# HKUST-Aerial-Robotics/ESVO

Measured on AMD Instinct MI355X. Metric: mapped events/sec (stereo TS raster + block matching + LM depth refinement + fusion), events resident in HBM before the timed region; exactly K ticks between two synchronisations, i.e. including the fill and the drain of the two-deep tick pipeline (`sustained`: the same workload over 1600 ticks), higher is better.
Workload: dtype f64

## Files before the change

### esvo_amd/csrc/api_core.hip

```cpp
#include "context.hpp"

namespace esvo_host {
thread_local std::string g_create_error;
}

namespace {

void invert3x3(const double* P, double* Kinv, double* Kinv_t) {
  const double a = P[0], b = P[1], cc = P[2], d = P[4], e = P[5], f = P[6], g = P[8], hh = P[9], i = P[10];
  const double det = a * (e * i - f * hh) - b * (d * i - f * g) + cc * (d * hh - e * g);
  const double id = 1.0 / det;
  Kinv[0] = (e * i - f * hh) * id; Kinv[1] = (cc * hh - b * i) * id; Kinv[2] = (b * f - cc * e) * id;
  Kinv[3] = (f * g - d * i) * id;  Kinv[4] = (a * i - cc * g) * id;  Kinv[5] = (cc * d - a * f) * id;
  Kinv[6] = (d * hh - e * g) * id; Kinv[7] = (b * g - a * hh) * id;  Kinv[8] = (a * e - b * d) * id;
  for (int r = 0; r < 3; ++r) Kinv_t[r] = (Kinv[r * 3 + 0] * P[3] + Kinv[r * 3 + 1] * P[7]) + Kinv[r * 3 + 2] * P[11];
}

int validate_params(const esvo_params_t* p, std::string& why) {
  if (p->ls_norm != ESVO_LSNORM_TDIST && p->ls_norm != ESVO_LSNORM_L2) { why = "LSnorm must be Tdist or l2 (DepthProblemSolver.cpp:121-131 exits on anything else)"; return ESVO_ERR_UNSUPPORTED; }
  if (p->bm_step < 1) { why = "BM_step must be >= 1"; return ESVO_ERR_INVALID_ARG; }
  if (p->patch_size_x < 1 || p->patch_size_x > 64 || p->patch_size_y < 1 || p->patch_size_y > 40) { why = "patch size must be within 1..64 x 1..40"; return ESVO_ERR_UNSUPPORTED; }
  if (p->median_blur_kernel_size < 0 || p->median_blur_kernel_size > 3) { why = "median_blur_kernel_size must be 0..3 (kernel 2k + 1)"; return ESVO_ERR_UNSUPPORTED; }
  if (p->max_event_queue_len < 0 || p->max_event_queue_len > TSQ_LMAX) { why = "max_event_queue_len must be 0 (one stamp per pixel) or 1..32"; return ESVO_ERR_UNSUPPORTED; }
  if (p->bm_max_disparity < p->bm_min_disparity || p->bm_min_disparity < 0) { why = "bad disparity range"; return ESVO_ERR_INVALID_ARG; }
// ... 20 lines not shown
  const double td_stdvar = std::sqrt(p.td_nu / (p.td_nu - 2) * (p.td_scale * p.td_scale));
  d.td_stdvar2 = td_stdvar * td_stdvar;
  d.lm_max_iter = p.lm_max_iteration; d.lm_maxfev = p.lm_max_iteration * 3;
  d.invdepth_min = p.invdepth_min; d.invdepth_max = p.invdepth_max;
  d.var_thr = p.stdvar_vis_threshold * p.stdvar_vis_threshold;
  d.cost_thr = (p.residual_vis_threshold * p.residual_vis_threshold) * (double)(p.patch_size_x * p.patch_size_y);
  d.age_thr = p.age_vis_threshold;
  d.fusion_radius = p.fusion_radius;
  d.reg_radius = p.reg_radius; d.reg_min_nb = p.reg_min_neighbours; d.reg_min_close = p.reg_min_close_neighbours;
  d.num_threads = p.num_threads;
  d.ls_norm = p.ls_norm;
}

template <typename T>
hipError_t dalloc(T** p, size_t n) { return hipMalloc(reinterpret_cast<void**>(p), (n ? n : 1) * sizeof(T)); }

void set_compute_band(esvo_context* h) {
  const int halo = 2 + (h->prm.regularization ? h->prm.reg_radius : 0);
  h->dp.cband_y0 = std::max(0, h->dp.band_y0 - halo);
  h->dp.cband_y1 = std::min(h->H, h->dp.band_y1 + halo);
}

void release_routing(esvo_context* h) {
  for (int cam = 0; cam < 2; ++cam) {
    if (h->h_route_ev[cam]) hipHostFree(h->h_route_ev[cam]);
    h->h_route_ev[cam] = nullptr;
    h->route_cap[cam] = 0;
  }
  if (h->h_route_gidx) hipHostFree(h->h_route_gidx);
  h->h_route_gidx = nullptr;
// ... 224 lines not shown
  CK(hipMalloc(reinterpret_cast<void**>(&h->d_map), map_buffer_bytes(npx)));
  CK(hipMalloc(reinterpret_cast<void**>(&h->d_map2), map_buffer_bytes(npx)));
  CK(hipMemset(h->d_map, 0, map_buffer_bytes(npx)));
  CK(hipMemset(h->d_map2, 0, map_buffer_bytes(npx)));
  h->d_map_cur = h->d_map;
  CK(dalloc(&h->d_owner_max, npx));
  CK(dalloc(&h->d_owner_min, npx));
  CK(dalloc(&h->d_own_w, E));
  CK(dalloc(&h->d_lkeep, E));
  h->codes_bytes = (E + 7) / 8 * 8;
  CK(dalloc(&h->d_codes, h->codes_bytes));
  CK(dalloc(&h->d_sel, E));
  CK(dalloc(&h->d_evmap, npx + 64));
  CK(dalloc(&h->d_reg_ab, npx));
  CK(dalloc(&h->d_reg_cd, npx));
  CK(dalloc(&h->d_exp_flags, npx));
  CK(dalloc(&h->d_exp_prefix, npx));
  CK(dalloc(&h->d_export, npx));
  CK(dalloc(&h->d_export_cell, npx));
  for (int i = 0; i < EV_N; ++i) CK(hipEventCreate(&h->evt[i]));
  if (h->tl_on) { CK(hipEventCreate(&h->tl_ref)); CK(hipEventRecord(h->tl_ref, h->stream)); CK(hipEventSynchronize(h->tl_ref)); }
  h->evt_ok = true;
  CK(hipEventCreateWithFlags(&h->evt_trk_read, hipEventDisableTiming));
  for (int cam = 0; cam < 2; ++cam) CK(hipEventCreateWithFlags(&h->evt_ingest[cam], hipEventDisableTiming));
  CK(hipHostMalloc(reinterpret_cast<void**>(&h->h_pose_pool), sizeof(double) * 16 * (size_t)h->max_poses * esvo_context::POSE_POOL));
  for (int i = 0; i < esvo_context::POSE_POOL; ++i) CK(hipEventCreate(&h->pool_evt[i]));
  h->pool_ok = true;
  for (int i = 0; i < 16; ++i) h->T_world_obs[i] = h->T_world_frame[i] = (i % 5 == 0) ? 1.0 : 0.0;
#undef CK
  *out = h;
// ... 4 lines not shown
  if (!h) return ESVO_OK;
  hipSetDevice(h->device);
  if (h->stream) hipStreamSynchronize(h->stream);
  if (h->stream_l) hipStreamSynchronize(h->stream_l);
  if (h->stream_l1) hipStreamSynchronize(h->stream_l1);
  if (h->stream_b) hipStreamSynchronize(h->stream_b);
  comm_release(h);
  em_release(h);
  void* ptrs[] = {h->d_lut, h->d_mask, h->d_fixmap[0], h->d_fixmap[1], h->d_sae[0], h->d_sae[1], h->d_raw, h->d_raw1, h->d_fwd_lut[0], h->d_fwd_lut[1], h->d_fwd_off[0], h->d_fwd_off[1],
                  h->d_fwd_src[0], h->d_fwd_src[1], h->d_fwd_val, h->d_ts[0],
                  h->d_ts[1], h->d_ring[0], h->d_ring[1], h->d_obs2[0][0], h->d_obs2[0][1], h->d_obs2[1][0], h->d_obs2[1][1], h->d_obs_tmp,
                  h->d_pose_T2[0], h->d_pose_T2[1], h->d_scan_tmp_b, h->d_cnt_b, h->d_tick_ev, h->d_match_slots, h->d_match_flags, h->d_match_prefix,
                  h->d_matches2[0], h->d_matches2[1], h->d_scan_tmp_l2[0], h->d_scan_tmp_l2[1], h->d_pt_slots2[0], h->d_pt_slots2[1], h->d_pt_flags2[0], h->d_pt_flags2[1], h->d_pt_prefix2[0], h->d_pt_prefix2[1], h->d_pts_tmp, h->d_stage[0], h->d_stage[1], h->d_counters2[0], h->d_counters2[1], h->d_scan_tmp,
                  h->d_win, h->d_frame_pose_T, h->d_fr_table, h->d_prop, h->d_tile_pts, h->d_tile_count, h->d_over_pts,
                  h->d_cell_count, h->d_cell_offset, h->d_cell_list, h->d_fuse_ctr, h->d_rec_ids, h->d_map, h->d_map2, h->d_owner_max, h->d_owner_min, h->d_exp_flags,
                  h->d_exp_prefix, h->d_export, h->d_export_cell, h->d_reg_ab, h->d_reg_cd, h->d_tsq[0], h->d_tsq[1], h->d_tsq_tcount, h->d_tsq_tlist, h->d_tsq_over, h->d_tsq_over_count, h->d_own_w, h->d_lkeep, h->d_codes, h->d_codes_send, h->d_codes_all, h->d_pts_send, h->d_pts_all, h->d_rank_kept,
                  h->d_sel, h->d_evmap, h->d_lm_fvec0, h->d_lm_fnorm0, h->d_lm_meta, h->d_lm_order, h->d_lm_hist, h->d_clk, h->d_ring_gidx, h->d_halo_viol, h->d_dn_flags, h->d_merge_a, h->d_merge_b, h->d_merge_plan, h->d_tsq_dup};
  for (void* p : ptrs) if (p) hipFree(p);
  if (h->h_counters) hipHostFree(h->h_counters);
  if (h->h_cnt_b) hipHostFree(h->h_cnt_b);
  if (h->h_pin) hipHostFree(h->h_pin);
  if (h->h_fr_table) hipHostFree(h->h_fr_table);
  if (h->evt_ok) for (int i = 0; i < EV_N; ++i) hipEventDestroy(h->evt[i]);
  if (h->pool_ok) for (int i = 0; i < esvo_context::POSE_POOL; ++i) hipEventDestroy(h->pool_evt[i]);
  if (h->h_pose_pool) hipHostFree(h->h_pose_pool);
  if (h->h_trk_ne) hipHostFree(h->h_trk_ne);
  if (h->h_trk_xyz) hipHostFree(h->h_trk_xyz);
  release_routing(h);
  for (int cam = 0; cam < 2; ++cam) if (h->d_wire[cam]) hipFree(h->d_wire[cam]);
  if (h->evt_trk_read) hipEventDestroy(h->evt_trk_read);
  if (h->tl_ref) hipEventDestroy(h->tl_ref);
// ... 101 lines not shown
    const u32 need = params->fusion_strategy == ESVO_FUSION_CONST_POINTS ? (u32)(1.5 * params->max_fusion_points) + 4u
                                                                         : (u32)params->max_fusion_frames + 2u;
    if (need > h->max_frames) FAIL(ESVO_ERR_CAPACITY, "fusion window (frames) exceeds the capacity fixed at esvo_create");
  }
  if (h->routed && (params->smooth_time_surface != h->prm.smooth_time_surface || params->median_blur_kernel_size != h->prm.median_blur_kernel_size ||
                    params->patch_size_y != h->prm.patch_size_y || params->denoising != h->prm.denoising || params->bm_updown))
    FAIL(ESVO_ERR_STATE, "the handle routes events by row (esvo_shard_set_routing): SmoothTimeSurface, median_blur_kernel_size, patch_size_Y and Denoising "
                         "fix the rows it renders and the events it keeps; esvo_reset + esvo_shard_set_routing to change them");
  esvo_params_t np = *params;
  np.max_events_per_tick = h->prm.max_events_per_tick;
  np.max_window_points = h->prm.max_window_points;
  np.max_poses_per_tick = h->prm.max_poses_per_tick;
  np.event_ring_capacity = h->prm.event_ring_capacity;
  if (np.max_event_queue_len != h->prm.max_event_queue_len) FAIL(ESVO_ERR_CAPACITY, "max_event_queue_len is fixed at esvo_create (the per-pixel queues are allocated there)");
  h->prm = np;
  fill_dev_params(h);
  set_compute_band(h);
  return ESVO_OK;
}

int esvo_set_stream(esvo_handle h, void* hip_stream) {
  if (!h) return ESVO_ERR_INVALID_ARG;
  API_LOCK(h);
  std::lock_guard<std::mutex> lp0(h->mu_push[0]), lp1(h->mu_push[1]);
  { int rcp = flush_pending_tick(h); if (rcp) return rcp; }
  HIPCHK(hipStreamSynchronize(h->stream));
  HIPCHK(hipStreamSynchronize(h->stream_l)); HIPCHK(hipStreamSynchronize(h->stream_l1));
  HIPCHK(hipStreamSynchronize(h->stream_b));
  if (h->own_stream && h->stream) hipStreamDestroy(h->stream);
  h->stream = reinterpret_cast<hipStream_t>(hip_stream);
// ... 107 lines not shown
```

### esvo_amd/csrc/api_map.hip

```cpp
#include <chrono>

#include "context.hpp"

namespace esvo_host {

u64 lower_bound_sec(const esvo_context* h, int cam, double t) {
  const auto& v = h->ts_host[cam];
  size_t lo = 0, hi = v.size();
  while (lo < hi) {
    size_t mid = (lo + hi) / 2;
    if (ns_to_sec(v[mid]) < t) lo = mid + 1; else hi = mid;
  }
  return h->ring_base[cam] + lo;
}
u64 ros_time_from_sec(double t) {
  long long sec64 = (long long)std::floor(t);
  u32 sec = (u32)sec64;
  u32 nsec = (u32)std::round((t - sec) * 1e9);
  sec += (nsec / 1000000000ul);
  nsec %= 1000000000ul;
  return (u64)sec * 1000000000ull + nsec;
}

int upload_poses(esvo_context* h, const uint64_t* pose_t_ns, const double* pose_T, size_t m, u32* d_zero_row = nullptr) {
// ... 347 lines not shown
  if (total > h->win_cap) {
    for (int e : tail_ev) if (e >= 0) hipEventRecord(h->evt[e], sb);
    FAIL(ESVO_ERR_CAPACITY, "window points exceed capacity");
  }
  const int o = par * EV_BACK_STRIDE;
  const bool timed = h->stage_events_on;
  h->back_timed[par] = timed;
  if (timed) hipEventRecord(h->evt[EV_FU0 + o], sb);
  launch_fuse(a, h->dp, sb);
  if (timed) hipEventRecord(h->evt[EV_FU1 + o], sb);
  h->d_map_cur = h->d_map;
  const bool do_clean = naive ? false : (h->prm.clean_requires_full_window ? (h->n_window_frames >= (size_t)h->prm.max_fusion_frames) : true);
  if (do_clean) launch_clean(h->d_map, h->dp, sb);
  if (timed) hipEventRecord(h->evt[EV_CL1 + o], sb);
  if (h->prm.regularization && !naive) {
    launch_reg_view(h->d_map, h->d_map2, h->d_owner_max, h->d_owner_min, h->d_reg_ab, h->d_reg_cd, h->d_cnt_b + 7, h->dp, sb);
    const u64 band_cells = (u64)std::max(h->dp.band_y1 - h->dp.band_y0, 1) * (u64)h->W;
    const bool sparse = h->reg_sparse_forced >= 0 ? h->reg_sparse_forced == 1 : (u64)h->stats.last_map_size * 10u < band_cells;
    launch_reg_apply(h->d_map, h->d_map2, h->d_owner_max, h->d_owner_min, h->d_reg_ab, h->d_reg_cd, h->d_cnt_b + 7, h->dp, sb, sparse);
    h->d_map_cur = h->d_map2;
  }
  HIPCHK(hipMemcpyAsync(h->h_cnt_b + 8 * par, h->d_cnt_b, sizeof(u32) * 8, hipMemcpyDeviceToHost, sb));
  if (h->routed) HIPCHK(hipMemcpyAsync(h->h_cnt_b + 8 * 3 + par, h->d_halo_viol, sizeof(u32), hipMemcpyDeviceToHost, sb));
  hipEventRecord(h->evt[EV_RG1 + o], sb);
  for (int e : tail_ev) if (e >= 0) hipEventRecord(h->evt[e], sb);
  HIPCHK(hipGetLastError());
  h->back_pending[par] = true;
  return ESVO_OK;
}

int export_map(esvo_context* h, std::vector<esvo_depth_point_t>& out, std::vector<u32>* cells) {
  launch_map_compact(h->d_map_cur, h->d_exp_flags, h->d_exp_prefix, h->d_cnt_b + 5, h->d_scan_tmp_b, h->d_export,
                     h->d_export_cell, h->dp, h->stream_b);
  int rc = read_counters_b(h, 2, true);
// ... 1394 lines not shown
```

### esvo_amd/csrc/common.hpp

```cpp
#pragma once

#include <hip/hip_runtime.h>
#include <stdint.h>

#include "../../include/esvo_hip.h"

#define ESVO_WAVE 64

#include <cstdlib>
#include <cstring>
inline const char* esvo_dev_switch(const char* name) {
  const char* on = std::getenv("ESVO_DEV_SWITCHES");
  return (on && std::strcmp(on, "1") == 0) ? std::getenv(name) : nullptr;
}

namespace esvo {

typedef unsigned long long u64;
typedef unsigned int u32;

struct CamConst {
  double P[12];
  double Kinv[9];
  double Kinv_t[3];
// ... 284 lines not shown
  u32* class_count;
  u32* class_total;
  u32 lds_cap;
  u32 pmax_plus1;
  u32* d_total;
  MapCell* map;
  u32* d_num_fusion;
  u32* n_touched;
  int naive;
  u32* owner_max;
  u32* owner_min;
  u32* n_reg_elems;
};
void launch_fuse(const FuseArgs& a, const DevParams& p, hipStream_t s);
void launch_clean(MapCell* map, const DevParams& p, hipStream_t s);
void launch_reg_view(const MapCell* map_in, MapCell* map_out, u32* owner_max, u32* owner_min, double2* ab, double2* cd,
                     u32* n_elems, const DevParams& p, hipStream_t s);
void launch_reg_apply(const MapCell* map_in, MapCell* map_out, const u32* owner_max, const u32* owner_min, const double2* ab,
                      const double2* cd, u32* n_elems, const DevParams& p, hipStream_t s, bool sparse = false);
struct SgmScratch {
  uint8_t *sobL, *rawL, *sobR, *rawR;
  int16_t* vol[6];
  int16_t *d1, *d1b;
  u32* d2key;
};
void launch_sgbm(const uint8_t* left, const uint8_t* right, const SgmScratch& s, int16_t* disp, int W, int H, hipStream_t st);
void launch_sgm_points(const esvo_event_t* ring, u64 first, u64 cap, u32 n, const float2* lut, const int16_t* disp, DevPoint* slots,
                       u32* flags, const DevParams& p, hipStream_t st);
void launch_sgm_naive(const DevPoint* pts, u32 n, const double* d_T_frame_obs, u32* owner, u32* pair_flags, u32* pair_rank, u32* d_total,
                      u32* scan_tmp, MapCell* map, const DevParams& p, hipStream_t st);
void launch_debug_image(const MapCell* map, u32* owner, uint8_t* bgr, const uint8_t* jet, int type, double max_range,
                        double min_range, double thr1, double thr2, const DevParams& p, hipStream_t s);
void launch_map_compact(const MapCell* map, u32* flags, u32* prefix, u32* d_total, u32* scan_tmp,
                        esvo_depth_point_t* out, u32* out_cell, const DevParams& p, hipStream_t s);
// ... 3 lines not shown
```

### esvo_amd/csrc/context.hpp

```cpp
#pragma once
#include <algorithm>
#include <array>
#include <atomic>
#include <chrono>
#include <cmath>
#include <cstdio>
#include <cstdlib>
#include <cstring>
#include <deque>
#include <mutex>
#include <string>
#include <vector>

#include "common.hpp"

using namespace esvo;

enum { EV_SC0 = 0, EV_SC1, EV_R1, EV_SC0b, EV_SC1b, EV_R1b, EV_FRAME,
       EV_T0, EV_BM0, EV_BM1, EV_S1, EV_LM0, EV_LM1, EV_S2, EV_CNT, EV_STG, EV_A1, EV_T0b, EV_BM0b, EV_BM1b, EV_S1b, EV_LM0b, EV_LM1b, EV_S2b, EV_CNTb, EV_STGb, EV_A1b,
       EV_FU0, EV_FU1, EV_CL1, EV_RG1, EV_POSE, EV_FU0b, EV_FU1b, EV_CL1b, EV_RG1b, EV_POSEb, EV_N };
constexpr int EV_BACK_STRIDE = EV_FU0b - EV_FU0;
constexpr int EV_FRONT_STRIDE = EV_T0b - EV_T0;
constexpr int EV_TS_STRIDE = EV_SC0b - EV_SC0;

// ... 240 lines not shown
  bool tick_pending = false;
  u64 committed_t_ns = 0;
  int tsq_len = 0;
  u64* d_tsq[2] = {nullptr, nullptr};
  u32* d_tsq_tcount = nullptr;
  uint4* d_tsq_tlist = nullptr;
  uint4* d_tsq_over = nullptr;
  u32* d_tsq_over_count = nullptr;
  u32 tsq_tcap = 0;
  static constexpr u64 TSQ_ROUND = 1ull << 20;
  u64 sh_first = 0;
  u64 sh_first_prev = 0;
  u64 em_guard_lo[2] = {~0ull, ~0ull};
  double2* d_reg_ab = nullptr;
  double2* d_reg_cd = nullptr;
  double T_world_frame[16];
  u32* d_exp_flags = nullptr;
  u32* d_exp_prefix = nullptr;
  esvo_depth_point_t* d_export = nullptr;
  u32* d_export_cell = nullptr;

  hipStream_t stream_t = nullptr;
  uint8_t* d_trk_blur = nullptr;
  uint8_t* d_trk_neg = nullptr;
  int16_t* d_trk_du = nullptr;
  int16_t* d_trk_dv = nullptr;
  float* d_trk_xyz = nullptr;
  double* d_trk_pts = nullptr;
  double* d_trk_out = nullptr;
  double* h_trk_ne = nullptr;
// ... 129 lines not shown
```

### esvo_amd/csrc/dev_hooks.hpp

```cpp
#pragma once
#if defined(LM_STATS) || defined(REG_STATS) || defined(ESVO_PERTURB_ONE_ULP)
#include "../../tools/dev_hooks/hooks_impl.hpp"
#endif
#ifndef LM_STATS
#define DEV_LM_EVAL(pr) do {} while (0)
#define DEV_LM_SHORTCUT(pr) do {} while (0)
#define DEV_LM_PROBLEM_FIELDS
#define DEV_LM_SET_SLOT(pr, s) do {} while (0)
#define DEV_LM_FIRST_EVAL_KNZ(pr, knz) do {} while (0)
#define DEV_LM_SCALE_ITER(pr) do {} while (0)
#define DEV_LM_JAC_DECL
#define DEV_LM_JAC_PASS(pr, active, x) do {} while (0)
#endif
#ifndef ESVO_PERTURB_ONE_ULP
#define DEV_PERTURB_POINT(o, s) do {} while (0)
#endif
#ifndef REG_STATS
#define DEV_REG_DECL
#define DEV_REG_BLOCK_BEGIN() do {} while (0)
#define DEV_REG_ROW_BEGIN(nclose)
#define DEV_REG_ROW_END(nclose) do {} while (0)
#define DEV_REG_BLOCK_END(lane, wv) do {} while (0)
#define DEV_REG_DONE(t, lane, nclose) do {} while (0)
#endif
```

### esvo_amd/csrc/kernels_fuse.hip

```cpp
#include <algorithm>
#include <type_traits>
#define DEV_HOOKS_FUSE_TU
#include "common.hpp"
#include "dev_hooks.hpp"
#include "fdiv.hpp"
#include "scan.hpp"

namespace esvo {

#ifndef BACK_WAVES
#define BACK_WAVES 6
#endif
#ifndef FUSE_WAVES
#define FUSE_WAVES 1
#endif

__device__ inline bool boundaryCheck(double x, double y, int W, int H) {
  return !(x < 0 || x >= (double)W || y < 0 || y >= (double)H);
}

__device__ inline bool fusion_cell(u32 prow, u32 pcol, int k, int radius, int W, int H, int& row, int& col) {
  int dy, dx;
  if (radius == 0) { dy = k >> 1; dx = k & 1; }
  else { dy = k / 3 - 1; dx = k % 3 - 1; }
// ... 583 lines not shown
  const bool valid = c.inv_depth > -1e-6 && (double)c.age >= p.age_thr && c.variance <= p.var_thr &&
                     c.inv_depth <= p.invdepth_max && c.inv_depth >= p.invdepth_min;
  if (valid) return;
  atomicAnd(&mf[cell], ~(CELL_ALIVE | CELL_GRID));
  const u32 b = c.row * (u32)p.W + c.col;
  if (b != (u32)cell && c.row < (u32)p.H && c.col < (u32)p.W) atomicAnd(&mf[b], ~CELL_GRID);
}
void launch_clean(MapCell* map, const DevParams& p, hipStream_t s) {
  const int ncell = p.W * p.H;
  hipLaunchKernelGGL(clean_kernel, dim3((ncell + 255) / 256), dim3(256), 0, s, map, p);
}

__global__ void __launch_bounds__(256) reg_view_kernel(const MapCell* __restrict__ map, MapCell* __restrict__ out,
                                                       double2* __restrict__ ab, double2* __restrict__ cd,
                                                       u32* __restrict__ owner_max, u32* __restrict__ owner_min,
                                                       u32* __restrict__ n_elems, int ncell, int W,
                                                       int band0, int band1, int view0, int view1, int l2) {
  const int cell = blockIdx.x * blockDim.x + threadIdx.x;
  bool alive = false;
  if (cell < ncell) {
    const u32 fl = map_flags(map, ncell)[cell];
    const int row = cell / W;
    if (row >= view0 && row < view1) {
      const double nan = __longlong_as_double(0x7ff8000000000000ll);
      double2 vab = make_double2(nan, nan);
      if (fl & CELL_ALIVE) {
        const MapCell& n = map[cell];
        const u32 b = n.row * (u32)W + n.col;
        atomicMax(&owner_max[b], n.seq + 1u);
        atomicMin(&owner_min[b], n.seq);
        if ((fl & CELL_GRID) && n.inv_depth > -1e-6) {
          vab = make_double2(n.inv_depth, 2.0 * sqrt(n.variance));
          cd[cell] = l2 ? make_double2(n.variance, 0.0) : make_double2(n.nu, n.scale2);
        }
      }
      ab[cell] = vab;
    }
    if (row >= band0 && row < band1) {
      alive = (fl & CELL_ALIVE) != 0;
      if (!alive) map_flags(out, ncell)[cell] = 0;
    }
  }
  const u64 am = __ballot(alive);
  if (n_elems && (threadIdx.x & 63) == 0 && am) atomicAdd(n_elems, (u32)__popcll(am));
}

#define REG_TX 64
#ifndef REG_TY
#define REG_TY 8
#endif
#ifndef REG_RB
#define REG_RB 4
#endif
#define REG_MARGIN 1
#define REG_MAXW 128
static_assert((REG_TX * REG_TY) % 64 == 0 && REG_TX == 64, "a wave is a tile row");
template <int RT, bool SPARSE = false>
__global__ void __launch_bounds__(REG_TX * REG_TY, BACK_WAVES) reg_apply_kernel(const MapCell* __restrict__ map, MapCell* __restrict__ out,
                                                                    const u32* __restrict__ owner_max,
                                                                    const u32* __restrict__ owner_min,
                                                                    const double2* __restrict__ ab,
                                                                    const double2* __restrict__ cd, DevParams p, u32* __restrict__ n_elems) {
  constexpr int NW = REG_TY;
  constexpr int UNITS = 4 * REG_RB;
  constexpr int UPW = (UNITS + NW - 1) / NW;
  __shared__ double2 s_ab[2][REG_RB][REG_MAXW];
  __shared__ double2 s_cd[2][REG_RB][REG_MAXW];
  __shared__ u64 s_vb[2][REG_RB][2];
  __shared__ u32 s_elem[REG_TX * REG_TY];
  __shared__ u32 s_wcount[REG_TY + 1];
  const int t = threadIdx.x, lane = t & 63, wv = t >> 6;
  const int tiles_x = (p.W + REG_TX - 1) / REG_TX;
  const int tile_c0 = (int)(blockIdx.x % tiles_x) * REG_TX, tile_r0 = (int)(blockIdx.x / tiles_x) * REG_TY;
  const int R = RT > 0 ? RT : p.reg_radius, Wn = 2 * R + 1;
  const int cr = tile_r0 + wv, cc = tile_c0 + lane;
  bool alive = false;
  if (cr < p.H && cc < p.W && cr >= p.band_y0 && cr < p.band_y1) alive = (map_flags(map, p.W * p.H)[cr * p.W + cc] & CELL_ALIVE) != 0;
// ... 16 lines not shown
    row = (int)c.row; col = (int)c.col;
    inv = c.inv_depth;
    sd_self2 = 2.0 * sqrt(c.variance);
    seq = c.seq;
  }
  const u32 b = (u32)row * (u32)p.W + (u32)col;
  const bool owner = has && owner_max[b] == seq + 1u;
  bool scan = owner && inv > -1e-6 && row >= R && col >= R;
  const int sc0 = tile_c0 - REG_MARGIN - R, sr0 = tile_r0 - REG_MARGIN - R;
  const int sw = REG_TX + 2 * (R + REG_MARGIN), sh = REG_TY + 2 * (R + REG_MARGIN);
  const int off = col - R - sc0;
  bool slow = scan && (off < 0 || off + Wn > sw || row - R < sr0 || row + R >= sr0 + sh);
  if (slow) scan = false;
  const u64 wmask = (Wn >= 64) ? ~0ull : ((1ull << Wn) - 1ull);
  u32 nb = 0, nclose = 0;
  double nu_post = 0, inv_post = 0, s2_post = 0, nu_div = 0;
  Recip rnu = make_recip(1.0);
  bool first = true;
  auto fuse_step = [&](double inv_obs, double nu_obs, double s2_obs) {
    if (first) {
      first = false;
      nu_post = nu_obs; inv_post = inv_obs; s2_post = s2_obs;
      nu_div = nu_post + 1;
      rnu = make_recip(nu_div);
      return;
    }
    const double nu_prior = nu_post, inv_prior = inv_post, s2_prior = s2_post;
    nu_post = (nu_obs < nu_prior) ? nu_obs : nu_prior;
    if (nu_post + 1 != nu_div) { nu_div = nu_post + 1; rnu = make_recip(nu_div); }
    const double ssum = s2_obs + s2_prior;
    const Recip rsum = make_recip(ssum);
    const double a1 = s2_obs * inv_prior + s2_prior * inv_obs;
    const double dd = inv_prior - inv_obs;
    const double a2 = dd * dd;
    const double pp = s2_prior * s2_obs;
    const double q1 = div_fast(a1, rsum);
    const double a3 = nu_post + div_fast(a2, rsum);
    const double a4 = div_fast(a3, rnu) * pp;
    const double q4 = div_fast(a4, rsum);
    const bool ok = (int)rnu.fast & (int)fdiv_ok_b4(ssum, a1, a2, a3, a4);
    if (ok) {
      inv_post = q1;
      s2_post = q4;
    } else {
      inv_post = a1 / ssum;
      s2_post = ((nu_post + a2 / ssum) / (nu_post + 1) * pp) / ssum;
    }
  };
  const double nan = __longlong_as_double(0x7ff8000000000000ll);
  double2 ld[UPW];
  const int n_blk = (sh + REG_RB - 1) / REG_RB;
  auto fetch_block = [&](int k) {
#pragma unroll
    for (int j = 0; j < UPW; ++j) {
      const int u = wv + NW * j;
      ld[j] = make_double2(nan, nan);
      if (u < UNITS && k < n_blk) {
        const int r = u >> 2, a = (u >> 1) & 1, hf = u & 1;
        const int y = k * REG_RB + r, sj = hf * 64 + lane;
        const int gy = sr0 + y, gx = sc0 + sj;
        if (sj < sw && y < sh && gy >= 0 && gy < p.H && gx >= 0 && gx < p.W) ld[j] = (a ? cd : ab)[gy * p.W + gx];
      }
    }
// ... 2 lines not shown
#pragma unroll
    for (int j = 0; j < UPW; ++j) {
      const int u = wv + NW * j;
      if (u < UNITS) {
        const int r = u >> 2, a = (u >> 1) & 1, hf = u & 1;
        const int sj = hf * 64 + lane;
        (a ? s_cd : s_ab)[buf][r][sj] = ld[j];
        if (!a) {
          const u64 vm = __ballot(sj < sw && ld[j].x == ld[j].x);
          if (lane == 0) s_vb[buf][r][hf] = vm;
        }
      }
    }
  };
  DEV_REG_DECL
  fetch_block(0);
  store_block(0);
  fetch_block(1);
  __syncthreads();
  for (int k = 0; k < n_blk; ++k) {
    const int buf = k & 1;
    DEV_REG_BLOCK_BEGIN();
#pragma unroll 1
    for (int r = 0; r < REG_RB; ++r) {
      const int gy = sr0 + k * REG_RB + r;
      DEV_REG_ROW_BEGIN(nclose)
      if (scan && gy >= row - R && gy <= row + R) {
        const u64 w0 = s_vb[buf][r][0], w1 = s_vb[buf][r][1];
        u64 bits = (off < 64) ? (w0 >> off) : 0ull;
        if (off > 0 && off < 64) bits |= w1 << (64 - off);
        if (off >= 64) bits = w1 >> (off - 64);
        bits &= wmask;
        nb += (u32)__popcll(bits);
        u32 cm2[2] = {0u, 0u};
        if (bits) {
          u32 lo = 0, hi = 0;
          const double2* tap = &s_ab[buf][r][off];
// ... 15 lines not shown
            for (int dc = 0; dc < 2 * RT + 1; ++dc) {
              const double2 q = tap[dc];
              const bool close = fabs(inv - q.x) < fmax(sd_self2, q.y);
              if (dc < 32) lo |= close ? (1u << dc) : 0u; else hi |= close ? (1u << (dc - 32)) : 0u;
            }
          } else {
            for (int dc = 0; dc < Wn; ++dc) {
              const double2 q = tap[dc];
              const bool close = fabs(inv - q.x) < fmax(sd_self2, q.y);
              if (dc < 32) lo |= close ? (1u << dc) : 0u; else hi |= close ? (1u << (dc - 32)) : 0u;
            }
          }
          cm2[0] = lo; cm2[1] = hi;
        }
        nclose += (u32)__popc(cm2[0]) + (u32)__popc(cm2[1]);
#pragma unroll 1
        for (int half = 0; half < 2; ++half) {
          u32 m = half ? cm2[1] : cm2[0];
          const int o2 = off + 32 * half;
          while (m) {
            const int kk = __builtin_ctz(m);
            m &= m - 1u;
            const double2 qa = s_ab[buf][r][o2 + kk], qc = s_cd[buf][r][o2 + kk];
            fuse_step(qa.x, qc.x, qc.y);
          }
        }
      }
      DEV_REG_ROW_END(nclose);
    }
    DEV_REG_BLOCK_END(lane, wv);
    if (k + 1 < n_blk) store_block(buf ^ 1);
    fetch_block(k + 2);
    __syncthreads();
  }
  DEV_REG_DONE(t, lane, nclose);
  if (slow) {
    for (int r = row - R; r <= row + R && r < p.H; ++r)
      for (int c2 = col - R; c2 <= col + R && c2 < p.W; ++c2) {
        const double2 q = ab[r * p.W + c2];
        if (!(q.x == q.x)) continue;
        nb++;
        const double diff = fabs(inv - q.x);
        if (diff < sd_self2 || diff < q.y) {
          nclose++;
          const double2 qc = cd[r * p.W + c2];
          fuse_step(q.x, qc.x, qc.y);
        }
      }
  }
  if (!has) return;
  u32* of = map_flags(out, p.W * p.H);
  if (!owner) { of[cell] = 0; return; }
  MapCell c = map[cell];
  if (c.inv_depth > -1e-6)
    c.inv_depth = (nb > (u32)p.reg_min_nb && nclose > (u32)p.reg_min_close) ? inv_post : -1.0;
  c.seq = owner_min[b];
  out[cell] = c;
  of[cell] = CELL_ALIVE | CELL_GRID;
}

__global__ void __launch_bounds__(256) reg_apply_l2_kernel(const MapCell* __restrict__ map, MapCell* __restrict__ out,
                                                           const u32* __restrict__ owner_max, const u32* __restrict__ owner_min,
                                                           const double2* __restrict__ ab, const double2* __restrict__ cd, DevParams p) {
  const int cell = blockIdx.x * blockDim.x + threadIdx.x;
  if (cell >= p.W * p.H) return;
  { const int r0 = cell / p.W; if (r0 < p.band_y0 || r0 >= p.band_y1) return; }
  if (!(map_flags(map, p.W * p.H)[cell] & CELL_ALIVE)) return;
  MapCell c = map[cell];
  u32* of = map_flags(out, p.W * p.H);
  const int row = (int)c.row, col = (int)c.col, R = p.reg_radius;
  const u32 b = (u32)row * (u32)p.W + (u32)col;
  if (owner_max[b] != c.seq + 1u) { of[cell] = 0; return; }
  if (c.inv_depth > -1e-6) {
// ... 16 lines not shown
      for (int r = row - R; r <= row + R && r < p.H; ++r)
        for (int c2 = col - R; c2 <= col + R && c2 < p.W; ++c2) {
          const double2 q = ab[r * p.W + c2];
          if (!(q.x == q.x)) continue;
          const double diff = fabs(c.inv_depth - q.x);
          if (diff < sd_self2 || diff < q.y) mean += q.x * (1.0 / cd[r * p.W + c2].x) / total;
        }
    c.inv_depth = set ? mean : -1.0;
  }
  c.seq = owner_min[b];
  out[cell] = c;
  of[cell] = CELL_ALIVE | CELL_GRID;
}

void launch_reg_view(const MapCell* map_in, MapCell* map_out, u32* owner_max, u32* owner_min, double2* ab, double2* cd,
                     u32* n_elems, const DevParams& p, hipStream_t s) {
  const int ncell = p.W * p.H;
  const int nb = (ncell + 255) / 256;
  if (p.ls_norm != ESVO_LSNORM_L2) n_elems = nullptr;
  hipLaunchKernelGGL(reg_view_kernel, dim3(nb), dim3(256), 0, s, map_in, map_out, ab, cd, owner_max, owner_min, n_elems, ncell, p.W,
                     p.band_y0, p.band_y1, p.cband_y0, p.cband_y1, p.ls_norm == ESVO_LSNORM_L2 ? 1 : 0);
}
void launch_reg_apply(const MapCell* map_in, MapCell* map_out, const u32* owner_max, const u32* owner_min, const double2* ab,
                      const double2* cd, u32* n_elems, const DevParams& p, hipStream_t s, bool sparse) {
  if (p.ls_norm == ESVO_LSNORM_L2) {
    const int ncell = p.W * p.H;
    hipLaunchKernelGGL(reg_apply_l2_kernel, dim3((ncell + 255) / 256), dim3(256), 0, s, map_in, map_out, owner_max, owner_min, ab, cd, p);
    return;
  }
  const int tiles_x = (p.W + REG_TX - 1) / REG_TX;
  const int ty0 = p.band_y0 / REG_TY, ty1 = (p.band_y1 + REG_TY - 1) / REG_TY;
  if (ty1 <= ty0) return;
  const int tiles_y = (p.H + REG_TY - 1) / REG_TY;
  const dim3 grid(tiles_x * tiles_y), block(REG_TX * REG_TY);
  if (sparse) {
    if (p.reg_radius == 20) hipLaunchKernelGGL((reg_apply_kernel<20, true>), grid, block, 0, s, map_in, map_out, owner_max, owner_min, ab, cd, p, n_elems);
    else if (p.reg_radius == 5) hipLaunchKernelGGL((reg_apply_kernel<5, true>), grid, block, 0, s, map_in, map_out, owner_max, owner_min, ab, cd, p, n_elems);
    else hipLaunchKernelGGL((reg_apply_kernel<0, true>), grid, block, 0, s, map_in, map_out, owner_max, owner_min, ab, cd, p, n_elems);
    return;
  }
  if (p.reg_radius == 20) hipLaunchKernelGGL(reg_apply_kernel<20>, grid, block, 0, s, map_in, map_out, owner_max, owner_min, ab, cd, p, n_elems);
  else if (p.reg_radius == 5) hipLaunchKernelGGL(reg_apply_kernel<5>, grid, block, 0, s, map_in, map_out, owner_max, owner_min, ab, cd, p, n_elems);
  else hipLaunchKernelGGL(reg_apply_kernel<0>, grid, block, 0, s, map_in, map_out, owner_max, owner_min, ab, cd, p, n_elems);
}

__global__ void __launch_bounds__(256) map_flags_kernel(const MapCell* __restrict__ map, u32* __restrict__ flags, int ncell, int W,
                                                        int band0, int band1) {
  const int cell = blockIdx.x * blockDim.x + threadIdx.x;
  if (cell >= ncell) return;
  const int row = cell / W;
  flags[cell] = (row >= band0 && row < band1 && (map_flags(map, ncell)[cell] & CELL_ALIVE)) ? 1u : 0u;
}
__global__ void __launch_bounds__(256) map_export_kernel(const MapCell* __restrict__ map, const u32* __restrict__ flags,
                                                         const u32* __restrict__ prefix, esvo_depth_point_t* __restrict__ out,
                                                         u32* __restrict__ out_cell, int ncell) {
  const int cell = blockIdx.x * blockDim.x + threadIdx.x;
  if (cell >= ncell || !flags[cell]) return;
  const MapCell& c = map[cell];
// ... 21 lines not shown
```

Measured before the change: 156.5 million.

## Split regularization fusion walk into a class-sorted follow-up kernel

The per-cell sequential Student-t fusion over close neighbours is taken out of the tiled reg_apply kernel. The tiled kernel now only records per-row close-neighbour bitmasks and bins the qualifying cells into classes by neighbour count. A new reg_walk kernel then processes each class with 64-lane waves, heaviest classes first, and prefetches the next tap. The aim is to remove wave divergence from lanes that have very different neighbour counts. The cost is extra HBM scratch of (2R+1) u64 words per pixel, mask writes and reads, atomics, and one more kernel launch per tick.

```diff
diff --git a/esvo_amd/csrc/api_core.hip b/esvo_amd/csrc/api_core.hip
--- a/esvo_amd/csrc/api_core.hip
+++ b/esvo_amd/csrc/api_core.hip
@@ -58,6 +58,24 @@
 
 template <typename T>
 hipError_t dalloc(T** p, size_t n) { return hipMalloc(reinterpret_cast<void**>(p), (n ? n : 1) * sizeof(T)); }
+
+hipError_t reg_walk_reserve(esvo_context* h) {
+  if (!h->prm.regularization || h->prm.ls_norm == ESVO_LSNORM_L2) return hipSuccess;
+  const size_t npx = (size_t)h->W * (size_t)h->H;
+  hipError_t e = hipSuccess;
+  if (!h->reg_walk.cls_cnt) {
+    if ((e = dalloc(&h->reg_walk.cls_cnt, (size_t)REG_NCLS)) != hipSuccess) return e;
+    if ((e = dalloc(&h->reg_walk.cls_list, (size_t)REG_NCLS * npx)) != hipSuccess) return e;
+    if ((e = dalloc(&h->reg_walk.row_bits, npx)) != hipSuccess) return e;
+  }
+  const int rows = 2 * h->prm.reg_radius + 1;
+  if (rows > h->reg_walk_rows) {
+    if (h->reg_walk.rmask) { hipFree(h->reg_walk.rmask); h->reg_walk.rmask = nullptr; h->reg_walk_rows = 0; }
+    if ((e = dalloc(&h->reg_walk.rmask, (size_t)rows * npx)) != hipSuccess) return e;
+    h->reg_walk_rows = rows;
+  }
+  return hipSuccess;
+}
 
 void set_compute_band(esvo_context* h) {
   const int halo = 2 + (h->prm.regularization ? h->prm.reg_radius : 0);
@@ -312,6 +330,7 @@
   CK(dalloc(&h->d_evmap, npx + 64));
   CK(dalloc(&h->d_reg_ab, npx));
   CK(dalloc(&h->d_reg_cd, npx));
+  CK(reg_walk_reserve(h));
   CK(dalloc(&h->d_exp_flags, npx));
   CK(dalloc(&h->d_exp_prefix, npx));
   CK(dalloc(&h->d_export, npx));
@@ -346,7 +365,7 @@
                   h->d_matches2[0], h->d_matches2[1], h->d_scan_tmp_l2[0], h->d_scan_tmp_l2[1], h->d_pt_slots2[0], h->d_pt_slots2[1], h->d_pt_flags2[0], h->d_pt_flags2[1], h->d_pt_prefix2[0], h->d_pt_prefix2[1], h->d_pts_tmp, h->d_stage[0], h->d_stage[1], h->d_counters2[0], h->d_counters2[1], h->d_scan_tmp,
                   h->d_win, h->d_frame_pose_T, h->d_fr_table, h->d_prop, h->d_tile_pts, h->d_tile_count, h->d_over_pts,
                   h->d_cell_count, h->d_cell_offset, h->d_cell_list, h->d_fuse_ctr, h->d_rec_ids, h->d_map, h->d_map2, h->d_owner_max, h->d_owner_min, h->d_exp_flags,
-                  h->d_exp_prefix, h->d_export, h->d_export_cell, h->d_reg_ab, h->d_reg_cd, h->d_tsq[0], h->d_tsq[1], h->d_tsq_tcount, h->d_tsq_tlist, h->d_tsq_over, h->d_tsq_over_count, h->d_own_w, h->d_lkeep, h->d_codes, h->d_codes_send, h->d_codes_all, h->d_pts_send, h->d_pts_all, h->d_rank_kept,
+                  h->d_exp_prefix, h->d_export, h->d_export_cell, h->d_reg_ab, h->d_reg_cd, h->reg_walk.rmask, h->reg_walk.row_bits, h->reg_walk.cls_cnt, h->reg_walk.cls_list, h->d_tsq[0], h->d_tsq[1], h->d_tsq_tcount, h->d_tsq_tlist, h->d_tsq_over, h->d_tsq_over_count, h->d_own_w, h->d_lkeep, h->d_codes, h->d_codes_send, h->d_codes_all, h->d_pts_send, h->d_pts_all, h->d_rank_kept,
                   h->d_sel, h->d_evmap, h->d_lm_fvec0, h->d_lm_fnorm0, h->d_lm_meta, h->d_lm_order, h->d_lm_hist, h->d_clk, h->d_ring_gidx, h->d_halo_viol, h->d_dn_flags, h->d_merge_a, h->d_merge_b, h->d_merge_plan, h->d_tsq_dup};
   for (void* p : ptrs) if (p) hipFree(p);
   if (h->h_counters) hipHostFree(h->h_counters);
@@ -478,6 +497,7 @@
   np.event_ring_capacity = h->prm.event_ring_capacity;
   if (np.max_event_queue_len != h->prm.max_event_queue_len) FAIL(ESVO_ERR_CAPACITY, "max_event_queue_len is fixed at esvo_create (the per-pixel queues are allocated there)");
   h->prm = np;
+  HIPCHK(reg_walk_reserve(h));
   fill_dev_params(h);
   set_compute_band(h);
   return ESVO_OK;
diff --git a/esvo_amd/csrc/api_map.hip b/esvo_amd/csrc/api_map.hip
--- a/esvo_amd/csrc/api_map.hip
+++ b/esvo_amd/csrc/api_map.hip
@@ -385,10 +385,10 @@
   if (do_clean) launch_clean(h->d_map, h->dp, sb);
   if (timed) hipEventRecord(h->evt[EV_CL1 + o], sb);
   if (h->prm.regularization && !naive) {
-    launch_reg_view(h->d_map, h->d_map2, h->d_owner_max, h->d_owner_min, h->d_reg_ab, h->d_reg_cd, h->d_cnt_b + 7, h->dp, sb);
+    launch_reg_view(h->d_map, h->d_map2, h->d_owner_max, h->d_owner_min, h->d_reg_ab, h->d_reg_cd, h->d_cnt_b + 7, h->reg_walk, h->dp, sb);
     const u64 band_cells = (u64)std::max(h->dp.band_y1 - h->dp.band_y0, 1) * (u64)h->W;
     const bool sparse = h->reg_sparse_forced >= 0 ? h->reg_sparse_forced == 1 : (u64)h->stats.last_map_size * 10u < band_cells;
-    launch_reg_apply(h->d_map, h->d_map2, h->d_owner_max, h->d_owner_min, h->d_reg_ab, h->d_reg_cd, h->d_cnt_b + 7, h->dp, sb, sparse);
+    launch_reg_apply(h->d_map, h->d_map2, h->d_owner_max, h->d_owner_min, h->d_reg_ab, h->d_reg_cd, h->d_cnt_b + 7, h->reg_walk, h->dp, sb, sparse);
     h->d_map_cur = h->d_map2;
   }
   HIPCHK(hipMemcpyAsync(h->h_cnt_b + 8 * par, h->d_cnt_b, sizeof(u32) * 8, hipMemcpyDeviceToHost, sb));
diff --git a/esvo_amd/csrc/common.hpp b/esvo_amd/csrc/common.hpp
--- a/esvo_amd/csrc/common.hpp
+++ b/esvo_amd/csrc/common.hpp
@@ -322,10 +322,17 @@
 };
 void launch_fuse(const FuseArgs& a, const DevParams& p, hipStream_t s);
 void launch_clean(MapCell* map, const DevParams& p, hipStream_t s);
+#define REG_NCLS 32
+struct RegWalk {
+  u64* rmask;
+  u64* row_bits;
+  u32* cls_cnt;
+  u32* cls_list;
+};
 void launch_reg_view(const MapCell* map_in, MapCell* map_out, u32* owner_max, u32* owner_min, double2* ab, double2* cd,
-                     u32* n_elems, const DevParams& p, hipStream_t s);
+                     u32* n_elems, const RegWalk& wk, const DevParams& p, hipStream_t s);
 void launch_reg_apply(const MapCell* map_in, MapCell* map_out, const u32* owner_max, const u32* owner_min, const double2* ab,
-                      const double2* cd, u32* n_elems, const DevParams& p, hipStream_t s, bool sparse = false);
+                      const double2* cd, u32* n_elems, const RegWalk& wk, const DevParams& p, hipStream_t s, bool sparse = false);
 struct SgmScratch {
   uint8_t *sobL, *rawL, *sobR, *rawR;
   int16_t* vol[6];
diff --git a/esvo_amd/csrc/context.hpp b/esvo_amd/csrc/context.hpp
--- a/esvo_amd/csrc/context.hpp
+++ b/esvo_amd/csrc/context.hpp
@@ -278,6 +278,8 @@
   u64 em_guard_lo[2] = {~0ull, ~0ull};
   double2* d_reg_ab = nullptr;
   double2* d_reg_cd = nullptr;
+  RegWalk reg_walk = {nullptr, nullptr, nullptr, nullptr};
+  int reg_walk_rows = 0;
   double T_world_frame[16];
   u32* d_exp_flags = nullptr;
   u32* d_exp_prefix = nullptr;
diff --git a/esvo_amd/csrc/dev_hooks.hpp b/esvo_amd/csrc/dev_hooks.hpp
--- a/esvo_amd/csrc/dev_hooks.hpp
+++ b/esvo_amd/csrc/dev_hooks.hpp
@@ -17,9 +17,10 @@
 #endif
 #ifndef REG_STATS
 #define DEV_REG_DECL
-#define DEV_REG_BLOCK_BEGIN() do {} while (0)
 #define DEV_REG_ROW_BEGIN(nclose)
-#define DEV_REG_ROW_END(nclose) do {} while (0)
-#define DEV_REG_BLOCK_END(lane, wv) do {} while (0)
-#define DEV_REG_DONE(t, lane, nclose) do {} while (0)
+#define DEV_REG_ROW_END(nclose, y) do {} while (0)
+#define DEV_REG_WALK_DECL
+#define DEV_REG_WALK_STEP() do {} while (0)
+#define DEV_REG_WALK_DONE(lane) do {} while (0)
+#define DEV_REG_DONE(t, lane, has, nclose) do {} while (0)
 #endif
diff --git a/esvo_amd/csrc/kernels_fuse.hip b/esvo_amd/csrc/kernels_fuse.hip
--- a/esvo_amd/csrc/kernels_fuse.hip
+++ b/esvo_amd/csrc/kernels_fuse.hip
@@ -621,7 +621,7 @@
 __global__ void __launch_bounds__(256) reg_view_kernel(const MapCell* __restrict__ map, MapCell* __restrict__ out,
                                                        double2* __restrict__ ab, double2* __restrict__ cd,
                                                        u32* __restrict__ owner_max, u32* __restrict__ owner_min,
-                                                       u32* __restrict__ n_elems, int ncell, int W,
+                                                       u32* __restrict__ n_elems, u32* __restrict__ cls_cnt, int ncell, int W,
                                                        int band0, int band1, int view0, int view1, int l2) {
   const int cell = blockIdx.x * blockDim.x + threadIdx.x;
   bool alive = false;
@@ -650,7 +650,49 @@
   }
   const u64 am = __ballot(alive);
   if (n_elems && (threadIdx.x & 63) == 0 && am) atomicAdd(n_elems, (u32)__popcll(am));
-}
+  if (cls_cnt && blockIdx.x == 0 && threadIdx.x < REG_NCLS) cls_cnt[threadIdx.x] = 0;
+}
+
+__device__ inline int reg_walk_class(u32 nclose, int Wn) {
+  const int c = (int)(sqrtf((float)nclose) * (float)REG_NCLS / (float)Wn);
+  return c < REG_NCLS - 1 ? c : REG_NCLS - 1;
+}
+
+struct RegFuse {
+  double nu_post = 0, inv_post = 0, s2_post = 0, nu_div = 0;
+  Recip rnu = make_recip(1.0);
+  bool first = true;
+  __device__ __forceinline__ void step(double inv_obs, double nu_obs, double s2_obs) {
+    if (first) {
+      first = false;
+      nu_post = nu_obs; inv_post = inv_obs; s2_post = s2_obs;
+      nu_div = nu_post + 1;
+      rnu = make_recip(nu_div);
+      return;
+    }
+    const double nu_prior = nu_post, inv_prior = inv_post, s2_prior = s2_post;
+    nu_post = (nu_obs < nu_prior) ? nu_obs : nu_prior;
+    if (nu_post + 1 != nu_div) { nu_div = nu_post + 1; rnu = make_recip(nu_div); }
+    const double ssum = s2_obs + s2_prior;
+    const Recip rsum = make_recip(ssum);
+    const double a1 = s2_obs * inv_prior + s2_prior * inv_obs;
+    const double dd = inv_prior - inv_obs;
+    const double a2 = dd * dd;
+    const double pp = s2_prior * s2_obs;
+    const double q1 = div_fast(a1, rsum);
+    const double a3 = nu_post + div_fast(a2, rsum);
+    const double a4 = div_fast(a3, rnu) * pp;
+    const double q4 = div_fast(a4, rsum);
+    const bool ok = (int)rnu.fast & (int)fdiv_ok_b4(ssum, a1, a2, a3, a4);
+    if (ok) {
+      inv_post = q1;
+      s2_post = q4;
+    } else {
+      inv_post = a1 / ssum;
+      s2_post = ((nu_post + a2 / ssum) / (nu_post + 1) * pp) / ssum;
+    }
+  }
+};
 
 #define REG_TX 64
 #ifndef REG_TY
@@ -667,7 +709,8 @@
                                                                     const u32* __restrict__ owner_max,
                                                                     const u32* __restrict__ owner_min,
                                                                     const double2* __restrict__ ab,
-                                                                    const double2* __restrict__ cd, DevParams p, u32* __restrict__ n_elems) {
+                                                                    const double2* __restrict__ cd, DevParams p, u32* __restrict__ n_elems,
+                                                                    RegWalk wk) {
   constexpr int NW = REG_TY;
   constexpr int UNITS = 4 * REG_RB;
   constexpr int UPW = (UNITS + NW - 1) / NW;
@@ -714,39 +757,8 @@
   if (slow) scan = false;
   const u64 wmask = (Wn >= 64) ? ~0ull : ((1ull << Wn) - 1ull);
   u32 nb = 0, nclose = 0;
-  double nu_post = 0, inv_post = 0, s2_post = 0, nu_div = 0;
-  Recip rnu = make_recip(1.0);
-  bool first = true;
-  auto fuse_step = [&](double inv_obs, double nu_obs, double s2_obs) {
-    if (first) {
-      first = false;
-      nu_post = nu_obs; inv_post = inv_obs; s2_post = s2_obs;
-      nu_div = nu_post + 1;
-      rnu = make_recip(nu_div);
-      return;
-    }
-    const double nu_prior = nu_post, inv_prior = inv_post, s2_prior = s2_post;
-    nu_post = (nu_obs < nu_prior) ? nu_obs : nu_prior;
-    if (nu_post + 1 != nu_div) { nu_div = nu_post + 1; rnu = make_recip(nu_div); }
-    const double ssum = s2_obs + s2_prior;
-    const Recip rsum = make_recip(ssum);
-    const double a1 = s2_obs * inv_prior + s2_prior * inv_obs;
-    const double dd = inv_prior - inv_obs;
-    const double a2 = dd * dd;
-    const double pp = s2_prior * s2_obs;
-    const double q1 = div_fast(a1, rsum);
-    const double a3 = nu_post + div_fast(a2, rsum);
-    const double a4 = div_fast(a3, rnu) * pp;
-    const double q4 = div_fast(a4, rsum);
-    const bool ok = (int)rnu.fast & (int)fdiv_ok_b4(ssum, a1, a2, a3, a4);
-    if (ok) {
-      inv_post = q1;
-      s2_post = q4;
-    } else {
-      inv_post = a1 / ssum;
-      s2_post = ((nu_post + a2 / ssum) / (nu_post + 1) * pp) / ssum;
-    }
-  };
+  RegFuse fz;
+  auto fuse_step = [&](double inv_obs, double nu_obs, double s2_obs) { fz.step(inv_obs, nu_obs, s2_obs); };
   const double nan = __longlong_as_double(0x7ff8000000000000ll);
   double2 ld[UPW];
   const int n_blk = (sh + REG_RB - 1) / REG_RB;
@@ -779,13 +791,14 @@
     }
   };
   DEV_REG_DECL
+  const int ncell = p.W * p.H;
+  u64 row_bits = 0;
   fetch_block(0);
   store_block(0);
   fetch_block(1);
   __syncthreads();
   for (int k = 0; k < n_blk; ++k) {
     const int buf = k & 1;
-    DEV_REG_BLOCK_BEGIN();
 #pragma unroll 1
     for (int r = 0; r < REG_RB; ++r) {
       const int gy = sr0 + k * REG_RB + r;
@@ -831,26 +844,19 @@
           cm2[0] = lo; cm2[1] = hi;
         }
         nclose += (u32)__popc(cm2[0]) + (u32)__popc(cm2[1]);
-#pragma unroll 1
-        for (int half = 0; half < 2; ++half) {
-          u32 m = half ? cm2[1] : cm2[0];
-          const int o2 = off + 32 * half;
-          while (m) {
-            const int kk = __builtin_ctz(m);
-            m &= m - 1u;
-            const double2 qa = s_ab[buf][r][o2 + kk], qc = s_cd[buf][r][o2 + kk];
-            fuse_step(qa.x, qc.x, qc.y);
-          }
-        }
-      }
-      DEV_REG_ROW_END(nclose);
-    }
-    DEV_REG_BLOCK_END(lane, wv);
+        if (cm2[0] | cm2[1]) {
+          const int j = gy - (row - R);
+          wk.rmask[(size_t)j * (size_t)ncell + (size_t)cell] = (u64)cm2[0] | ((u64)cm2[1] << 32);
+          row_bits |= 1ull << j;
+        }
+      }
+      DEV_REG_ROW_END(nclose, k * REG_RB + r);
+    }
     if (k + 1 < n_blk) store_block(buf ^ 1);
     fetch_block(k + 2);
     __syncthreads();
   }
-  DEV_REG_DONE(t, lane, nclose);
+  DEV_REG_DONE(t, lane, has, nclose);
   if (slow) {
     for (int r = row - R; r <= row + R && r < p.H; ++r)
       for (int c2 = col - R; c2 <= col + R && c2 < p.W; ++c2) {
@@ -865,15 +871,90 @@
         }
       }
   }
-  if (!has) return;
+  const bool walk = scan && nb > (u32)p.reg_min_nb && nclose > (u32)p.reg_min_close;
+  const int cls = reg_walk_class(nclose, Wn);
+  for (u64 todo = __ballot(walk); todo;) {
+    const int leader = __builtin_ctzll(todo);
+    const int lc = __shfl(cls, leader);
+    const u64 same = __ballot(walk && cls == lc);
+    u32 at = 0;
+    if (lane == leader) at = atomicAdd(&wk.cls_cnt[lc], (u32)__popcll(same));
+    at = (u32)__shfl((int)at, leader);
+    if (walk && cls == lc) {
+      wk.cls_list[(size_t)lc * (size_t)ncell + at + (u32)__popcll(same & ((1ull << lane) - 1ull))] = (u32)cell;
+      wk.row_bits[cell] = row_bits;
+    }
+    todo &= ~same;
+  }
+  if (!has || walk) return;
   u32* of = map_flags(out, p.W * p.H);
   if (!owner) { of[cell] = 0; return; }
   MapCell c = map[cell];
   if (c.inv_depth > -1e-6)
-    c.inv_depth = (nb > (u32)p.reg_min_nb && nclose > (u32)p.reg_min_close) ? inv_post : -1.0;
+    c.inv_depth = (nb > (u32)p.reg_min_nb && nclose > (u32)p.reg_min_close) ? fz.inv_post : -1.0;
   c.seq = owner_min[b];
   out[cell] = c;
   of[cell] = CELL_ALIVE | CELL_GRID;
+}
+
+__global__ void __launch_bounds__(64, BACK_WAVES) reg_walk_kernel(const MapCell* __restrict__ map, MapCell* __restrict__ out,
+                                                                  const u32* __restrict__ owner_min, const double2* __restrict__ ab,
+                                                                  const double2* __restrict__ cd, DevParams p, RegWalk wk) {
+  const int lane = threadIdx.x, ncell = p.W * p.H;
+  u32 first_wave = 0, idx = 0, n_cls = 0;
+  int cls = -1;
+  for (int c = REG_NCLS - 1; c >= 0; --c) {
+    const u32 n = wk.cls_cnt[c], nw = (n + 63u) >> 6;
+    if (blockIdx.x < first_wave + nw) { cls = c; n_cls = n; idx = (blockIdx.x - first_wave) * 64u + (u32)lane; break; }
+    first_wave += nw;
+  }
+  if (cls < 0) return;
+  const bool act = idx < n_cls;
+  DEV_REG_WALK_DECL
+  if (act) {
+    const int cell = (int)wk.cls_list[(size_t)cls * (size_t)ncell + idx];
+    MapCell c = map[cell];
+    const int R = p.reg_radius;
+    const int base0 = ((int)c.row - R) * p.W + ((int)c.col - R);
+    u64 rows = wk.row_bits[cell];
+    RegFuse fz;
+    u64 m = 0, m_next = 0;
+    int j_next = -1, base = 0;
+    auto load_next_row = [&]() {
+      if (rows) {
+        j_next = __builtin_ctzll(rows);
+        rows &= rows - 1ull;
+        m_next = wk.rmask[(size_t)j_next * (size_t)ncell + (size_t)cell];
+      } else j_next = -1;
+    };
+    auto next_tap = [&]() -> int {
+      if (m == 0) {
+        if (j_next < 0) return -1;
+        m = m_next; base = base0 + j_next * p.W;
+        load_next_row();
+      }
+      const int k = __builtin_ctzll(m);
+      m &= m - 1ull;
+      return base + k;
+    };
+    load_next_row();
+    int a = next_tap();
+    double q_inv = 0; double2 q_cd = make_double2(0, 0);
+    if (a >= 0) { q_inv = ab[a].x; q_cd = cd[a]; }
+    while (a >= 0) {
+      const double o_inv = q_inv; const double2 o_cd = q_cd;
+      a = next_tap();
+      if (a >= 0) { q_inv = ab[a].x; q_cd = cd[a]; }
+      DEV_REG_WALK_STEP();
+      fz.step(o_inv, o_cd.x, o_cd.y);
+    }
+    const u32 b = c.row * (u32)p.W + c.col;
+    c.inv_depth = fz.inv_post;
+    c.seq = owner_min[b];
+    out[cell] = c;
+    map_flags(out, ncell)[cell] = CELL_ALIVE | CELL_GRID;
+  }
+  DEV_REG_WALK_DONE(lane);
 }
 
 __global__ void __launch_bounds__(256) reg_apply_l2_kernel(const MapCell* __restrict__ map, MapCell* __restrict__ out,
@@ -920,15 +1001,15 @@
 }
 
 void launch_reg_view(const MapCell* map_in, MapCell* map_out, u32* owner_max, u32* owner_min, double2* ab, double2* cd,
-                     u32* n_elems, const DevParams& p, hipStream_t s) {
+                     u32* n_elems, const RegWalk& wk, const DevParams& p, hipStream_t s) {
   const int ncell = p.W * p.H;
   const int nb = (ncell + 255) / 256;
   if (p.ls_norm != ESVO_LSNORM_L2) n_elems = nullptr;
-  hipLaunchKernelGGL(reg_view_kernel, dim3(nb), dim3(256), 0, s, map_in, map_out, ab, cd, owner_max, owner_min, n_elems, ncell, p.W,
-                     p.band_y0, p.band_y1, p.cband_y0, p.cband_y1, p.ls_norm == ESVO_LSNORM_L2 ? 1 : 0);
+  hipLaunchKernelGGL(reg_view_kernel, dim3(nb), dim3(256), 0, s, map_in, map_out, ab, cd, owner_max, owner_min, n_elems,
+                     p.ls_norm != ESVO_LSNORM_L2 ? wk.cls_cnt : nullptr, ncell, p.W, p.band_y0, p.band_y1, p.cband_y0, p.cband_y1, p.ls_norm == ESVO_LSNORM_L2 ? 1 : 0);
 }
 void launch_reg_apply(const MapCell* map_in, MapCell* map_out, const u32* owner_max, const u32* owner_min, const double2* ab,
-                      const double2* cd, u32* n_elems, const DevParams& p, hipStream_t s, bool sparse) {
+                      const double2* cd, u32* n_elems, const RegWalk& wk, const DevParams& p, hipStream_t s, bool sparse) {
   if (p.ls_norm == ESVO_LSNORM_L2) {
     const int ncell = p.W * p.H;
     hipLaunchKernelGGL(reg_apply_l2_kernel, dim3((ncell + 255) / 256), dim3(256), 0, s, map_in, map_out, owner_max, owner_min, ab, cd, p);
@@ -940,14 +1021,16 @@
   const int tiles_y = (p.H + REG_TY - 1) / REG_TY;
   const dim3 grid(tiles_x * tiles_y), block(REG_TX * REG_TY);
   if (sparse) {
-    if (p.reg_radius == 20) hipLaunchKernelGGL((reg_apply_kernel<20, true>), grid, block, 0, s, map_in, map_out, owner_max, owner_min, ab, cd, p, n_elems);
-    else if (p.reg_radius == 5) hipLaunchKernelGGL((reg_apply_kernel<5, true>), grid, block, 0, s, map_in, map_out, owner_max, owner_min, ab, cd, p, n_elems);
-    else hipLaunchKernelGGL((reg_apply_kernel<0, true>), grid, block, 0, s, map_in, map_out, owner_max, owner_min, ab, cd, p, n_elems);
-    return;
-  }
-  if (p.reg_radius == 20) hipLaunchKernelGGL(reg_apply_kernel<20>, grid, block, 0, s, map_in, map_out, owner_max, owner_min, ab, cd, p, n_elems);
-  else if (p.reg_radius == 5) hipLaunchKernelGGL(reg_apply_kernel<5>, grid, block, 0, s, map_in, map_out, owner_max, owner_min, ab, cd, p, n_elems);
-  else hipLaunchKernelGGL(reg_apply_kernel<0>, grid, block, 0, s, map_in, map_out, owner_max, owner_min, ab, cd, p, n_elems);
+    if (p.reg_radius == 20) hipLaunchKernelGGL((reg_apply_kernel<20, true>), grid, block, 0, s, map_in, map_out, owner_max, owner_min, ab, cd, p, n_elems, wk);
+    else if (p.reg_radius == 5) hipLaunchKernelGGL((reg_apply_kernel<5, true>), grid, block, 0, s, map_in, map_out, owner_max, owner_min, ab, cd, p, n_elems, wk);
+    else hipLaunchKernelGGL((reg_apply_kernel<0, true>), grid, block, 0, s, map_in, map_out, owner_max, owner_min, ab, cd, p, n_elems, wk);
+  } else {
+    if (p.reg_radius == 20) hipLaunchKernelGGL(reg_apply_kernel<20>, grid, block, 0, s, map_in, map_out, owner_max, owner_min, ab, cd, p, n_elems, wk);
+    else if (p.reg_radius == 5) hipLaunchKernelGGL(reg_apply_kernel<5>, grid, block, 0, s, map_in, map_out, owner_max, owner_min, ab, cd, p, n_elems, wk);
+    else hipLaunchKernelGGL(reg_apply_kernel<0>, grid, block, 0, s, map_in, map_out, owner_max, owner_min, ab, cd, p, n_elems, wk);
+  }
+  const int band_cells = (p.band_y1 - p.band_y0) * p.W;
+  hipLaunchKernelGGL(reg_walk_kernel, dim3((band_cells + 63) / 64 + REG_NCLS), dim3(64), 0, s, map_in, map_out, owner_min, ab, cd, p, wk);
 }
 
 __global__ void __launch_bounds__(256) map_flags_kernel(const MapCell* __restrict__ map, u32* __restrict__ flags, int ncell, int W,
```

Result: slower. 154.2 million, median of 2 (-1.5%).
